# krullgit/3D-Object-Detection-for-autonomous-navigation

Measured on AMD Instinct MI355X. Metric: frames/sec (whole node) + p50 per-frame ms, 16k-pt pillars, higher is better.
Workload: dtype f32 (GEMMs on the 16-bit matrix pipe as split operands -- two float16 pieces per value, 3 products, fp32 accumulate: fp32-equivalent results, measured 1.5e-6 max from the fp32 oracle at this shape)

## Files before the change

3d-object-detection-for-autonomous-navigation_amd/csrc/backbone.hip:

```cpp
#include <stdio.h>
#include <stdlib.h>
#include <string.h>

#include "pp_common.h"

typedef float f32x16 __attribute__((ext_vector_type(16)));
typedef _Float16 f16x8 __attribute__((ext_vector_type(8)));
#define PC_MFMA(A, B, C) __builtin_amdgcn_mfma_f32_32x32x16_f16(A, B, C, 0, 0, 0)
#define PC_PRODUCTS(ACC, XH, XM, YH, YM) \
    ACC = PC_MFMA(XM, YH, ACC); ACC = PC_MFMA(XH, YM, ACC); ACC = PC_MFMA(XH, YH, ACC);
typedef unsigned u32x4 __attribute__((ext_vector_type(4)));

__device__ __forceinline__ float4 buf_load16(__amdgpu_buffer_rsrc_t r, unsigned voff, unsigned soff) {
    const u32x4 v = __builtin_amdgcn_raw_buffer_load_b128(r, voff, soff, 0);
    return make_float4(__uint_as_float(v.x), __uint_as_float(v.y), __uint_as_float(v.z), __uint_as_float(v.w));
}
__device__ __forceinline__ void buf_store16(float4 v, __amdgpu_buffer_rsrc_t r, unsigned voff, unsigned soff) {
    const u32x4 u = {__float_as_uint(v.x), __float_as_uint(v.y), __float_as_uint(v.z), __float_as_uint(v.w)};
    __builtin_amdgcn_raw_buffer_store_b128(u, r, voff, soff, 0);
}
__device__ __forceinline__ __amdgpu_buffer_rsrc_t make_rsrc(const void* base) {
    return __builtin_amdgcn_make_buffer_rsrc(const_cast<void*>(base), 0, 0x7ffffffe, 0x00020000);
}

// ... 464 lines not shown
                const int row = ((it0 + u) * 64 + lane) / ROW4;
                v[u] = *reinterpret_cast<const float4*>(so + row * OSTR + c4 * 4);
                op[u] = s_opix[wave * 32 + row];
            }
#pragma unroll
            for (int u = 0; u < 4; ++u) {
                const int row = ((it0 + u) * 64 + lane) / ROW4;
                if (p0 + wave * 32 + row < a.M)
                    *reinterpret_cast<float4*>(dst + (size_t)(op[u] + delta) * a.ld_out) = v[u];
            }
        }
    }
    if (a.head_mode != 0) {
        f32x16 hacc;
#pragma unroll
        for (int r = 0; r < 16; ++r) hacc[r] = 0.f;
        const float* hA = so + r32 * OSTR + h * (NT / 2);
        const float* hB = a.head_wt + (size_t)r32 * NT + h * (NT / 2);
#pragma unroll
        for (int q = 0; q < NT / 8; ++q) {
            const float4 av = *reinterpret_cast<const float4*>(hA + q * 4);
            const float4 bw = *reinterpret_cast<const float4*>(hB + q * 4);
            hacc = __builtin_amdgcn_mfma_f32_32x32x2f32(av.x, bw.x, hacc, 0, 0, 0);
            hacc = __builtin_amdgcn_mfma_f32_32x32x2f32(av.y, bw.y, hacc, 0, 0, 0);
            hacc = __builtin_amdgcn_mfma_f32_32x32x2f32(av.z, bw.z, hacc, 0, 0, 0);
            hacc = __builtin_amdgcn_mfma_f32_32x32x2f32(av.w, bw.w, hacc, 0, 0, 0);
        }
        const float hb = (a.head_mode == 1) ? a.head_bias[r32] : 0.f;
#pragma unroll
        for (int r = 0; r < 16; ++r) {
            const int prow = wave * 32 + (r & 3) + 8 * (r >> 2) + 4 * h;
            if (p0 + prow < a.M) {
                float* hp = a.head + (size_t)(s_opix[prow] + delta) * PP_HEAD_COLS + r32;
                float v = hacc[r] + hb;
                if (a.head_mode == 2) v += *hp;
                *hp = v;
            }
        }
    }
}


__device__ __forceinline__ float dpp_quad(float v, const int ctrl_xor1) {
    const int x = __float_as_int(v);
    return __int_as_float(ctrl_xor1 ? __builtin_amdgcn_mov_dpp(x, 0xB1, 0xf, 0xf, true)
                                    : __builtin_amdgcn_mov_dpp(x, 0x4E, 0xf, 0xf, true));
}
#define QUAD_XCH(A, B, BIT, XOR1)                          \
    {                                                      \
        const float t_ = (BIT) ? (A) : (B);                \
        const float u_ = dpp_quad(t_, XOR1);               \
        (A) = (BIT) ? u_ : (A);                            \
        (B) = (BIT) ? (B) : u_;                            \
    }
__device__ __forceinline__ void quad_transpose4(float& r0, float& r1, float& r2, float& r3, int lane) {
    const bool b0 = lane & 1, b1 = lane & 2;
    QUAD_XCH(r0, r1, b0, 1)
    QUAD_XCH(r2, r3, b0, 1)
    QUAD_XCH(r0, r2, b1, 0)
    QUAD_XCH(r1, r3, b1, 0)
}

typedef float f32x2_t __attribute__((ext_vector_type(2)));
typedef _Float16 f16x2_t __attribute__((ext_vector_type(2)));
__device__ __forceinline__ void split_f16x2(const float (&v)[8], f16x8& hi, f16x8& mid) {
#pragma unroll
    for (int j = 0; j < 8; j += 2) {
        const f32x2_t x = {v[j], v[j + 1]};
        const f16x2_t h = __builtin_convertvector(x, f16x2_t);
        const f32x2_t r1 = {v[j] - (float)h.x, v[j + 1] - (float)h.y};
        const f16x2_t m = __builtin_convertvector(r1, f16x2_t);
        hi[j] = h.x; hi[j + 1] = h.y;
        mid[j] = m.x; mid[j + 1] = m.y;
    }
}

__device__ __forceinline__ void fast_divmod(int n, int d, float inv_d, int& q, int& r) {
    q = (int)((float)n * inv_d);
    r = n - q * d;
    if (r < 0) { --q; r += d; }
    if (r >= d) { ++q; r -= d; }
}

template <int NT, int S, int WPS, int PREC, int OCC = 0, int TR = 0>
__global__ __launch_bounds__(256, WPS) void k_sep_u(GemmArgs a, int ntiles) {
    static_assert(TR == 0 || (PREC == 1 && OCC == 0), "training forward: split-precision, dense input");
    constexpr bool PW = TR == 2;
    constexpr int NTAP = (TR == 1) ? 11 : 9;
    constexpr int KCH = 16, LSTR = KCH + 4, G = 4;
    constexpr int WW = S + 3;
    constexpr int NLD = PW ? 2 : 3 * WW;
    constexpr int SAW = 32 * LSTR;
    constexpr int SB = (PREC == 0) ? NT * LSTR : PP_NPIECE * NT * 8;
    constexpr int NB4 = (PREC == 0) ? (NT * G + 255) / 256 : (NT * 2 * PP_NPIECE + 255) / 256;
    constexpr int NTILES = NT / 32;
    constexpr int KQ = KCH / 8;
    __shared__ __attribute__((aligned(16))) float smem[8 * SAW + 2 * SB + (PW ? 0 : NTAP * 256) + (TR ? 8 * NT : 0)];
    const int tid = threadIdx.x, lane = tid & 63, wave = tid >> 6;
    float* const sAw = smem + wave * 2 * SAW;
    float* const sB = smem + 8 * SAW;
    float* const sDW = smem + 8 * SAW + 2 * SB;
    [[maybe_unused]] float* const sST = smem + 8 * SAW + 2 * SB + (PW ? 0 : NTAP * 256);

    const int xcd = blockIdx.x & 7, gl = blockIdx.x >> 3, GL = gridDim.x >> 3;
    const int nt_ = ntiles - a.tile_lo;
    const int tbase = a.tile_lo + (int)(((long long)xcd * nt_) >> 3), tend = a.tile_lo + (int)(((long long)(xcd + 1) * nt_) >> 3);
    const int first = tbase + gl;
    const int n0 = blockIdx.y * NT;
    if (first >= tend) {
        if (TR && a.tr_stat != nullptr && tid < 2 * NT)
            a.tr_stat[((size_t)blockIdx.x * 2 + tid / NT) * a.n_total + n0 + tid % NT] = 0.f;
        if (TR && a.tr_stat != nullptr && tid == 0 && blockIdx.y == 0) a.tr_stat[(size_t)gridDim.x * 2 * a.n_total + blockIdx.x] = 0.f;
        return;
    }
    const int ntl = (tend - first + GL - 1) / GL;
    const int cin = a.cin;
    const int nchunks = cin / KCH;
    const int total = ntl * nchunks;

    const int c4 = lane & 3, q = lane >> 2;
    const __amdgpu_buffer_rsrc_t rs_in = make_rsrc(reinterpret_cast<const char*>(a.in) - (PW ? 0 : PP_ZPAD_FLOATS * 4));
    const __amdgpu_buffer_rsrc_t rs_wt = make_rsrc(PREC == 0 ? (const void*)a.wt : (const void*)a.wt16);
    const int hw = a.px_h * a.px_w;
    const float inv_hw = 1.0f / (float)hw, inv_w = 1.0f / (float)a.px_w;
    const int rs4 = a.in_w * cin * 4, cin4 = cin * 4;
    unsigned aoff[NLD];
    [[maybe_unused]] unsigned doff = 0x80000000u;
    [[maybe_unused]] const __amdgpu_buffer_rsrc_t rs_d = make_rsrc(TR ? (const void*)a.tr_D : (const void*)a.in);
    [[maybe_unused]] const bool d_out = TR && a.tr_D != nullptr && blockIdx.y == 0;
    [[maybe_unused]] const bool tr_act = TR && a.tr_coef != nullptr;
#define U_TILE_OFFSETS(TILE)                                                                             \
    {                                                                                                    \
        const int pix0_ = (TILE) * 128 + wave * 32 + 2 * q;                                              \
        const bool pvalid_ = pix0_ < a.M;                                                                \
        if (TR) doff = pvalid_ ? (unsigned)pix0_ * (unsigned)cin4 + (unsigned)(c4 * 16) : 0x80000000u;   \
        const int pc_ = pvalid_ ? pix0_ : 0;                                                             \
        if (PW) {    \
            aoff[0] = pvalid_ ? (unsigned)pc_ * (unsigned)cin4 + (unsigned)(c4 * 16) : 0x80000000u;      \
            aoff[NLD - 1] = pvalid_ ? aoff[0] + (unsigned)cin4 : 0x80000000u;                            \
        } else {                                                                                         \
        int b_, rem_, y_, x0_;                                                                           \
        fast_divmod(pc_, hw, inv_hw, b_, rem_);         \
        fast_divmod(rem_, a.px_w, inv_w, y_, x0_);                                                       \
        const int yi_ = y_ * S - 1, xi_ = x0_ * S - 1;                                                   \
        const unsigned cbase_ =                                                                          \
            (unsigned)(((b_ * a.in_h + y_ * S) * a.in_w + x0_ * S) * cin) * 4u + PP_ZPAD_FLOATS * 4u;    \
                        \
        bool rowok_[3], colok_[WW];                                                                      \
        unsigned rowoff_[3], coloff_[WW];                                                                \
        _Pragma("unroll") for (int dy_ = 0; dy_ < 3; ++dy_) {                                            \
            rowok_[dy_] = pvalid_ & ((unsigned)(yi_ + dy_) < (unsigned)a.in_h);                          \
            rowoff_[dy_] = cbase_ + (unsigned)((dy_ - 1) * rs4);                                         \
        }                                                                                                \
        _Pragma("unroll") for (int dx_ = 0; dx_ < WW; ++dx_) {                                           \
            colok_[dx_] = (unsigned)(xi_ + dx_) < (unsigned)a.in_w;                                      \
            coloff_[dx_] = (unsigned)((dx_ - 1) * cin4);                                                 \
        }                                                                                                \
                                                                       \
        unsigned wbits_[3] = {0u, 0u, 0u};                                                               \
        const bool bits_ = OCC && a.occbits != nullptr;                                     \
        if (bits_) {                                                                                     \
            const unsigned long long* ob_ = a.occbits + (size_t)b_ * a.in_h * a.occ_w64;                 \
            const int pos0_ = xi_ + 1, wi_ = pos0_ >> 6, sh_ = pos0_ & 63;                               \
            _Pragma("unroll") for (int dy_ = 0; dy_ < 3; ++dy_) {                                        \
                const int yy_ = min(max(yi_ + dy_, 0), a.in_h - 1);     \
                const unsigned long long* r_ = ob_ + (size_t)yy_ * a.occ_w64 + wi_;                      \
                const unsigned long long lo_ = r_[0], hi_ = r_[1];                                       \
                wbits_[dy_] = (unsigned)((lo_ >> sh_) | ((hi_ << 1) << (63 - sh_)));                     \
            }                                                                                            \
        }                                                                                                \
        _Pragma("unroll") for (int e = 0; e < NLD; ++e) {                                                \
            const int dy_ = e / WW, dx_ = e % WW;                                                        \
            bool ok_ = rowok_[dy_] & colok_[dx_];                                                        \
            if (OCC) {                                                                                   \
                if (bits_) {                                                                             \
                    ok_ = ok_ & (((wbits_[dy_] >> dx_) & 1u) != 0u);                                     \
                } else {                                                                                 \
                    bool occ_ = false;                                                                   \
                    const int cidx_ = ok_ ? (yi_ + dy_) * a.in_w + xi_ + dx_ : 0;                        \
                    for (int z_ = 0; z_ < a.occ_nz; ++z_)                                                \
                        occ_ = occ_ | (a.occ[(size_t)(b_ * a.occ_nz + z_) * (a.in_h * a.in_w) + cidx_] >= 0); \
                    ok_ = ok_ & occ_;                                                                    \
                }                                                                                        \
            }                                                                                            \
            aoff[e] = (ok_ ? rowoff_[dy_] + coloff_[dx_] : 0u) + (unsigned)(c4 * 16);                    \
        }                                                                                                \
        }                                                                                                \
    }
    constexpr int NBI = (PREC == 0) ? NT * G : NT * 2 * PP_NPIECE;
    unsigned boff[NB4];
    int bdst[NB4];
#pragma unroll
    for (int r = 0; r < NB4; ++r) {
        const int e_ = (tid + 256 * r) % NBI;
        if (PREC == 0) {
            boff[r] = (unsigned)(((n0 + e_ / G) * cin + (e_ % G) * 4) * 4);
            bdst[r] = (e_ / G) * LSTR + (e_ % G) * 4;
        } else {
            const int piece = e_ / (NT * 2), rem = e_ % (NT * 2), row = rem >> 1, half = rem & 1;
            boff[r] = (unsigned)(((piece * a.n_total + n0 + row) * 16 + half * 8) * 2);
            bdst[r] = piece * (NT * 8) + row * 8 + ((half ^ ((row >> 3) & 1)) * 4);
        }
    }
    const unsigned bstep = (PREC == 0) ? (unsigned)(KCH * 4) : (unsigned)(PP_NPIECE * a.n_total * 32);
    float4 rin[NLD];
    float4 rb0, rb1, rb2;
    rb0 = rb1 = rb2 = make_float4(0.f, 0.f, 0.f, 0.f);
    static_assert(NB4 <= 3, "weight prefetch registers");
#define U_LOAD_ACT(KCIDX, RIN)                                                                           \
    {                                                                                                    \
        const unsigned so_ = (unsigned)(KCIDX) * (KCH * 4);                                              \
        _Pragma("unroll") for (int e = 0; e < NLD; ++e) RIN[e] = buf_load16(rs_in, aoff[e], so_);        \
    }
#define U_LOAD_WT(KCIDX)                                                                                 \
    {                                                                                                    \
        const unsigned sb_ = (unsigned)(KCIDX) * bstep;                                                  \
        if (NBI % 256 == 0 || NB4 > 1 || tid < NBI) rb0 = buf_load16(rs_wt, boff[0], sb_);               \
        if (NB4 > 1 && (NBI >= 512 || tid + 256 < NBI)) rb1 = buf_load16(rs_wt, boff[NB4 > 1 ? 1 : 0], sb_);  \
        if (NB4 > 2 && (NBI >= 768 || tid + 512 < NBI)) rb2 = buf_load16(rs_wt, boff[NB4 > 2 ? 2 : 0], sb_);  \
    }
#define U_LOAD_CHUNK(KCIDX) { U_LOAD_ACT(KCIDX, rin) U_LOAD_WT(KCIDX) }
    int ld_tile = first, ld_kc = 0;
    int st_kc = 0;
    int mm_tile = first, mm_kc = 0;
    [[maybe_unused]] float st_n = 0.f;
    U_TILE_OFFSETS(ld_tile)
    U_LOAD_CHUNK(0)
    ld_kc = 1;
    {
        const int ngrp = cin / 4;
        if (!PW) for (int e = tid; e < 9 * ngrp; e += 256) {
            const int t = e / ngrp, g4 = e - t * ngrp;
            reinterpret_cast<float4*>(sDW)[g4 * NTAP + t] = reinterpret_cast<const float4*>(a.dw)[e];
        }
        if (TR) for (int e = tid; e < 8 * NT; e += 256) sST[e] = 0.f;
        if (tr_act) {
            for (int g4 = tid; g4 < ngrp; g4 += 256) {
                const float4 q0 = a.tr_coef[4 * g4], q1 = a.tr_coef[4 * g4 + 1], q2 = a.tr_coef[4 * g4 + 2], q3 = a.tr_coef[4 * g4 + 3];
                reinterpret_cast<float4*>(sDW)[g4 * NTAP + 9] = make_float4(q0.x, q1.x, q2.x, q3.x);
                reinterpret_cast<float4*>(sDW)[g4 * NTAP + 10] = make_float4(q0.y, q1.y, q2.y, q3.y);
            }
        }
    }

    f32x16 acc[NTILES];
#pragma unroll
    for (int n = 0; n < NTILES; ++n)
#pragma unroll
        for (int r = 0; r < 16; ++r) acc[n][r] = 0.f;
    const int h = lane >> 5, r32 = lane & 31;
    float bias_r[NTILES];
#pragma unroll
    for (int n = 0; n < NTILES; ++n) bias_r[n] = (TR && a.bias == nullptr) ? 0.f : a.bias[n0 + n * 32 + r32];
    __syncthreads();

#define U_MFMA(I)                                                                                        \
    if (PREC == 1) {                                                                                     \
        const float* cA = cA0 + ((I) & 1) * SAW;                                                         \
        const float* cB = cB0 + ((I) & 1) * SB;                                                          \
        const float4 a0 = *reinterpret_cast<const float4*>(cA), a1 = *reinterpret_cast<const float4*>(cA + 4);  \
        const float av[8] = {a0.x, a0.y, a0.z, a0.w, a1.x, a1.y, a1.z, a1.w};                            \
        f16x8 ah, am;                                                                                    \
        split_f16x2(av, ah, am);                                                                         \
        _Pragma("unroll") for (int n = 0; n < NTILES; ++n) {                                             \
            const f16x8 bh = *reinterpret_cast<const f16x8*>(cB + n * 32 * 8);                           \
            const f16x8 bm = *reinterpret_cast<const f16x8*>(cB + NT * 8 + n * 32 * 8);                  \
            PC_PRODUCTS(acc[n], ah, am, bh, bm)                                                          \
        }                                                                                                \
    }                                                                                                    \
    if (PREC == 0) {                                                                                     \
        const float* cA = sAw + ((I) & 1) * SAW + r32 * LSTR + h * (KCH / 2);                            \
        const float* cB = sB + ((I) & 1) * SB + r32 * LSTR + h * (KCH / 2);                              \
        float4 a4[KQ];                                                                                   \
        _Pragma("unroll") for (int qq = 0; qq < KQ; ++qq) a4[qq] = *reinterpret_cast<const float4*>(cA + qq * 4);  \
        _Pragma("unroll") for (int n = 0; n < NTILES; ++n) {                                             \
            float4 b4[KQ];                                                                               \
            _Pragma("unroll") for (int qq = 0; qq < KQ; ++qq) b4[qq] = *reinterpret_cast<const float4*>(cB + n * 32 * LSTR + qq * 4);  \
            _Pragma("unroll") for (int qq = 0; qq < KQ; ++qq) {                                          \
                acc[n] = __builtin_amdgcn_mfma_f32_32x32x2f32(a4[qq].x, b4[qq].x, acc[n], 0, 0, 0);      \
                acc[n] = __builtin_amdgcn_mfma_f32_32x32x2f32(a4[qq].y, b4[qq].y, acc[n], 0, 0, 0);      \
                acc[n] = __builtin_amdgcn_mfma_f32_32x32x2f32(a4[qq].z, b4[qq].z, acc[n], 0, 0, 0);      \
                acc[n] = __builtin_amdgcn_mfma_f32_32x32x2f32(a4[qq].w, b4[qq].w, acc[n], 0, 0, 0);      \
            }                                                                                            \
        }                                                                                                \
    }
#define U_STAGE2(P, RIN)                                                                                 \
    {                                                                                                    \
        constexpr int buf = (P) & 1;    \
        float4 o0 = make_float4(0.f, 0.f, 0.f, 0.f), o1 = o0;                                            \
        if (tr_act) {    \
            const float4 sc_ = *reinterpret_cast<const float4*>(twp + 36), sh_ = *reinterpret_cast<const float4*>(twp + 40);  \
            _Pragma("unroll") for (int e = 0; e < NLD; ++e) {                                            \
                RIN[e].x = fmaxf(fmaf(RIN[e].x, sc_.x, sh_.x), 0.f); RIN[e].y = fmaxf(fmaf(RIN[e].y, sc_.y, sh_.y), 0.f);  \
                RIN[e].z = fmaxf(fmaf(RIN[e].z, sc_.z, sh_.z), 0.f); RIN[e].w = fmaxf(fmaf(RIN[e].w, sc_.w, sh_.w), 0.f);  \
            }                                                                                            \
        }                                                                                                \
        if (PW) { o0 = RIN[0]; o1 = RIN[NLD - 1]; }                                                      \
        if (!PW) {                                                                                       \
            const float* tw = twp;                                                                       \
            _Pragma("unroll") for (int dy = 0; dy < 3; ++dy)                                             \
                _Pragma("unroll") for (int dx = 0; dx < 3; ++dx) {                                       \
                    const float4 w4 = *reinterpret_cast<const float4*>(tw + (dy * 3 + dx) * 4);          \
                    const float4 v0 = RIN[PW ? 0 : dy * WW + dx], v1 = RIN[PW ? 0 : dy * WW + S + dx];   \
                    o0.x = fmaf(v0.x, w4.x, o0.x); o0.y = fmaf(v0.y, w4.y, o0.y);                        \
                    o0.z = fmaf(v0.z, w4.z, o0.z); o0.w = fmaf(v0.w, w4.w, o0.w);                        \
                    o1.x = fmaf(v1.x, w4.x, o1.x); o1.y = fmaf(v1.y, w4.y, o1.y);                        \
                    o1.z = fmaf(v1.z, w4.z, o1.z); o1.w = fmaf(v1.w, w4.w, o1.w);                        \
                }                                                                                        \
        }                                                                                                \
        float* dA = sAw + buf * SAW + (2 * q) * LSTR + c4 * 4;                                           \
        *reinterpret_cast<float4*>(dA) = o0;                                                             \
        *reinterpret_cast<float4*>(dA + LSTR) = o1;                                                      \
        if (d_out) {        \
                                                                               \
            const unsigned dv_ = doff + (unsigned)st_kc * (KCH * 4);                                     \
            buf_store16(o0, rs_d, dv_, 0u);                                                              \
            buf_store16(o1, rs_d, dv_ + (unsigned)cin4, 0u);                                             \
        }                                                                                                \
        if (NBI % 256 == 0 || NB4 > 1 || tid < NBI) *reinterpret_cast<float4*>(sB + buf * SB + bdst[0]) = rb0;  \
        if (NB4 > 1 && (NBI >= 512 || tid + 256 < NBI)) *reinterpret_cast<float4*>(sB + buf * SB + bdst[NB4 > 1 ? 1 : 0]) = rb1;  \
        if (NB4 > 2 && (NBI >= 768 || tid + 512 < NBI)) *reinterpret_cast<float4*>(sB + buf * SB + bdst[NB4 > 2 ? 2 : 0]) = rb2;  \
        twp += 4 * (4 * NTAP);                                                                           \
        if (++st_kc == nchunks) { st_kc = 0; twp = sDW + c4 * (4 * NTAP); }                              \
    }
#define U_STAGE(P) U_STAGE2(P, rin)
#define U_ISSUE()                                                                                        \
    {                                                                                                    \
        if (ld_kc == 0) U_TILE_OFFSETS(ld_tile)                                                          \
        U_LOAD_CHUNK(ld_kc)                                                                              \
        if (++ld_kc == nchunks) { ld_kc = 0; ld_tile += GL; }                                            \
    }
#define U_ACT(X) (TR ? (X) : relu_keep_nan(X))
#define U_EPILOGUE()                                                                                     \
    {                                                                                                    \
        const int pw = mm_tile * 128 + wave * 32;                                                        \
        [[maybe_unused]] const int nw = min(max(a.M - pw, 0), 32);    \
        if (TR && nw > 0) {      \
            _Pragma("unroll") for (int n = 0; n < NTILES; ++n) {                                         \
                float s1 = 0.f;                                                                          \
                _Pragma("unroll") for (int r = 0; r < 16; ++r) s1 += acc[n][r];                          \
                s1 += __shfl_xor(s1, 32);                                                                \
                const float mean_ = s1 / (float)nw;                                                      \
                float q = 0.f;                                                                           \
                _Pragma("unroll") for (int r = 0; r < 16; ++r) {                                         \
                    const float dz = acc[n][r] - mean_;                                                  \
                    if (pw + (r & 3) + 8 * (r >> 2) + 4 * h < a.M) q = fmaf(dz, dz, q);                  \
                }                                                                                        \
                q += __shfl_xor(q, 32);                                                                  \
                if (h == 0) {    \
                    float n_ = st_n, s_ = sST[(wave * 2 + 0) * NT + n * 32 + r32], m_ = sST[(wave * 2 + 1) * NT + n * 32 + r32];  \
                    bn_chan_merge(n_, s_, m_, (float)nw, s1, q);                                         \
                    sST[(wave * 2 + 0) * NT + n * 32 + r32] = s_;                                        \
                    sST[(wave * 2 + 1) * NT + n * 32 + r32] = m_;                                        \
                }                                                                                        \
            }                                                                                            \
            st_n += (float)nw;                                                                           \
        }                                                                                                \
        if (pw < a.M) {                                                                                  \
            const int qi = lane & 3, qj = r32 >> 2;                                                      \
            float* dst = a.out + (size_t)(pw + 4 * h + qi) * a.ld_out + a.co_off + n0 + qj * 4;          \
            const bool full = pw + 32 <= a.M;              \
            const int ldo = a.ld_out;                                                                    \
            if (full) {                                                                                  \
                _Pragma("unroll") for (int n = 0; n < NTILES; ++n) {                                     \
                    const float bvn = bias_r[n];                                                         \
                    _Pragma("unroll") for (int g = 0; g < 4; ++g) {                                      \
                        float x0 = U_ACT(acc[n][4 * g + 0] + bvn), x1 = U_ACT(acc[n][4 * g + 1] + bvn);          \
                        float x2 = U_ACT(acc[n][4 * g + 2] + bvn), x3 = U_ACT(acc[n][4 * g + 3] + bvn);          \
                        quad_transpose4(x0, x1, x2, x3, lane);                                           \
                        *reinterpret_cast<float4*>(dst + (8 * g) * ldo + n * 32) = make_float4(x0, x1, x2, x3);  \
                    }                                                                                    \
                }                                                                                        \
            } else {                                                                                     \
                _Pragma("unroll") for (int n = 0; n < NTILES; ++n) {                                     \
                    const float bvn = bias_r[n];                                                         \
                    _Pragma("unroll") for (int g = 0; g < 4; ++g) {                                      \
                        float x0 = U_ACT(acc[n][4 * g + 0] + bvn), x1 = U_ACT(acc[n][4 * g + 1] + bvn);          \
                        float x2 = U_ACT(acc[n][4 * g + 2] + bvn), x3 = U_ACT(acc[n][4 * g + 3] + bvn);          \
                        quad_transpose4(x0, x1, x2, x3, lane);                                           \
                        if (pw + 8 * g + 4 * h + qi < a.M)                                               \
                            *reinterpret_cast<float4*>(dst + (8 * g) * ldo + n * 32) = make_float4(x0, x1, x2, x3);  \
                    }                                                                                    \
                }                                                                                        \
            }                                                                                            \
        }                                                                                                \
        _Pragma("unroll") for (int n = 0; n < NTILES; ++n)                                               \
            _Pragma("unroll") for (int r = 0; r < 16; ++r) acc[n][r] = 0.f;                              \
        mm_kc = 0;                                                                                       \
        mm_tile += GL;                                                                                   \
    }

    const float* twp = sDW + c4 * (4 * NTAP);
    const float* const cA0 = sAw + r32 * LSTR + h * (KCH / 2);
    const float* const cB0 = sB + r32 * 8 + ((h ^ ((r32 >> 3) & 1)) * 4);
    U_STAGE(0)
    U_ISSUE()
    __syncthreads();
    int i = 0;
    for (; i + 3 < total; i += 2) {
        U_MFMA(0)
        U_STAGE(1)
        U_ISSUE()
        if (++mm_kc == nchunks) U_EPILOGUE()
        __syncthreads();
        U_MFMA(1)
        U_STAGE(0)
        U_ISSUE()
        if (++mm_kc == nchunks) U_EPILOGUE()
        __syncthreads();
    }
    U_MFMA(0)
    U_STAGE(1)
    if (++mm_kc == nchunks) U_EPILOGUE()
    __syncthreads();
    U_MFMA(1)
    ++mm_kc;
    U_EPILOGUE()
    if (TR && a.tr_stat != nullptr) {
        __syncthreads();
        const float* red = sST;
        float wn[4] = {0.f, 0.f, 0.f, 0.f};
        for (int t = first; t < tend; t += GL)
#pragma unroll
            for (int w = 0; w < 4; ++w) wn[w] += (float)min(max(a.M - (t * 128 + w * 32), 0), 32);
        if (tid < NT) {
            float n_ = 0.f, s_ = 0.f, m_ = 0.f;
#pragma unroll
            for (int w = 0; w < 4; ++w) bn_chan_merge(n_, s_, m_, wn[w], red[(w * 2) * NT + tid], red[(w * 2 + 1) * NT + tid]);
            a.tr_stat[((size_t)blockIdx.x * 2 + 0) * a.n_total + n0 + tid] = s_;
            a.tr_stat[((size_t)blockIdx.x * 2 + 1) * a.n_total + n0 + tid] = m_;
        }
        if (tid == 0 && blockIdx.y == 0) a.tr_stat[(size_t)gridDim.x * 2 * a.n_total + blockIdx.x] = ((wn[0] + wn[1]) + wn[2]) + wn[3];
    }
#undef U_MFMA
#undef U_STAGE
#undef U_ISSUE
#undef U_EPILOGUE
#undef U_ACT
#undef U_LOAD_CHUNK
#undef U_TILE_OFFSETS
}

constexpr int SEP128_WPB = 2, SEP64_WPB = 3;
constexpr int sep_u_wpc(int nt, int s, bool prec) {
    return s == 1 ? (prec ? (nt == 128 ? SEP128_WPB : (nt == 64 ? SEP64_WPB : 3)) : (nt == 128 ? 3 : 4))
                  : (prec ? (nt == 128 ? 2 : 3) : (nt == 128 ? 2 : (nt == 64 ? 3 : 4)));
}

template <int NT, int S>
static void launch_u(const GemmArgs& a, int n_total, bool prec, bool occ, hipStream_t s) {
    constexpr int WPS = sep_u_wpc(NT, S, false), WPB = sep_u_wpc(NT, S, true);
    const int ntiles = (a.M + 127) / 128;
    const int ny = n_total / NT;
    int slots = (g_num_cus * (prec ? WPB : WPS)) / ny;
    const int mine = ntiles - a.tile_lo;
    int gx = mine < slots ? mine : slots;
    gx = (gx + 7) & ~7;
    dim3 grid((unsigned)gx, ny);
    if (occ)
        PP_LAUNCH("k_sep_u", (k_sep_u<NT, S, WPB, 1, 1>), grid, dim3(256), 0, s, a, ntiles);
    else if (prec)
        PP_LAUNCH("k_sep_u", (k_sep_u<NT, S, WPB, 1>), grid, dim3(256), 0, s, a, ntiles);
    else
        PP_LAUNCH("k_sep_u", (k_sep_u<NT, S, WPS, 0>), grid, dim3(256), 0, s, a, ntiles);
}

int launch_sep_train(const SepTrainArgs& t, hipStream_t s) {
    const long long M = (long long)t.batch * t.out_h * t.out_w;
    const long long in_bytes = (long long)t.batch * t.in_h * t.in_w * t.cin * 4;
    if (t.cin % KC != 0 || t.cout % 32 != 0 || (t.stride != 1 && t.stride != 2) || t.out_w % 2 != 0 || M >= (1 << 24) ||
        in_bytes >= (1ll << 31) - 4096 || M * t.cin * 4 >= (1ll << 31) - 4096 || t.cin > 256)
        return 0;
    GemmArgs a;
    memset(&a, 0, sizeof(a));
    a.in = t.in; a.dw = t.dw; a.wt16 = t.wt16; a.n_total = t.cout; a.out = t.Z;
    a.M = (int)M; a.in_h = t.in_h; a.in_w = t.in_w; a.cin = t.cin; a.px_h = t.out_h; a.px_w = t.out_w;
    a.stride = t.stride; a.ld_out = t.cout; a.co_off = 0; a.cout = t.cout;
    a.tr_coef = t.coef; a.tr_D = t.D; a.tr_stat = t.stat;
    const int ntiles = (a.M + 127) / 128;
    const int nt = (t.cout % 128 == 0) ? 128 : (t.cout % 64 == 0 ? 64 : 32);
    const int ny = t.cout / nt;
    const int wpb = (nt == 128) ? 2 : 3;
    int slots = (g_num_cus * wpb) / ny;
    int gx = ntiles < slots ? ntiles : slots;
    gx = (gx + 7) & ~7;
    const dim3 grid((unsigned)gx, ny);
    const char* tg = t.tag ? t.tag : "k_sep_u_tr";
    if (t.stride == 1) {
        if (nt == 128) PP_LAUNCH(tg, (k_sep_u<128, 1, 2, 1, 0, 1>), grid, dim3(256), 0, s, a, ntiles);
        else if (nt == 64) PP_LAUNCH(tg, (k_sep_u<64, 1, 3, 1, 0, 1>), grid, dim3(256), 0, s, a, ntiles);
        else PP_LAUNCH(tg, (k_sep_u<32, 1, 3, 1, 0, 1>), grid, dim3(256), 0, s, a, ntiles);
    } else {
        if (nt == 128) PP_LAUNCH(tg, (k_sep_u<128, 2, 2, 1, 0, 1>), grid, dim3(256), 0, s, a, ntiles);
        else if (nt == 64) PP_LAUNCH(tg, (k_sep_u<64, 2, 3, 1, 0, 1>), grid, dim3(256), 0, s, a, ntiles);
        else PP_LAUNCH(tg, (k_sep_u<32, 2, 3, 1, 0, 1>), grid, dim3(256), 0, s, a, ntiles);
    }
    return gx;
}

int launch_rows_train(const RowsTrainArgs& t, hipStream_t s) {
    const long long M = t.rows;
    if (t.K % KC != 0 || t.N % 32 != 0 || M % 2 != 0 || M >= (1 << 24) || M * t.K * 4 >= (1ll << 31) - 4096 || t.ld_out % 4 != 0)
        return 0;
    GemmArgs a;
    memset(&a, 0, sizeof(a));
    a.in = t.in; a.wt16 = t.wt16; a.n_total = t.N; a.out = t.out; a.bias = t.bias;
    a.M = (int)M; a.in_h = 1; a.in_w = (int)M; a.cin = t.K; a.px_h = 1; a.px_w = (int)M;
    a.stride = 1; a.ld_out = t.ld_out; a.co_off = 0; a.cout = t.N;
    a.tr_stat = t.stat;
    const int ntiles = (a.M + 127) / 128;
    const int nt = (t.N % 128 == 0) ? 128 : (t.N % 64 == 0 ? 64 : 32);
    const int ny = t.N / nt;
    const int wpb = 3;
    int slots = (g_num_cus * wpb) / ny;
    if (slots < 8) slots = 8;
    int gx = ntiles < slots ? ntiles : slots;
    gx = (gx + 7) & ~7;
    const dim3 grid((unsigned)gx, ny);
    const char* tg = t.tag ? t.tag : "k_sep_u_tr";
    if (nt == 128) PP_LAUNCH(tg, (k_sep_u<128, 1, 3, 1, 0, 2>), grid, dim3(256), 0, s, a, ntiles);
    else if (nt == 64) PP_LAUNCH(tg, (k_sep_u<64, 1, 3, 1, 0, 2>), grid, dim3(256), 0, s, a, ntiles);
    else PP_LAUNCH(tg, (k_sep_u<32, 1, 3, 1, 0, 2>), grid, dim3(256), 0, s, a, ntiles);
    return gx;
}

template <int CO>
__global__ __launch_bounds__(512, 1) void k_sep_p(GemmArgs a, int ntiles) {
    constexpr int KCH = 16, LSTR = KCH + 4, WW = 4, NLD = 12;
    constexpr int SAW = 32 * LSTR;
    constexpr int SB1 = PP_NPIECE * CO * 8;
    constexpr int NTILES = CO / 64;
    constexpr int NB4 = (2 * CO * 2 * PP_NPIECE) / 512;
    __shared__ __attribute__((aligned(16))) float smem[16 * SAW + 4 * SB1 + 9 * 256];
    const int tid = threadIdx.x, lane = tid & 63, wave = tid >> 6;
    const int pg = wave & 3, grp = wave >> 2;
    float* const sA = smem;
    float* const sB = smem + 16 * SAW;
    float* const sDW = smem + 16 * SAW + 4 * SB1;

    const int xcd = blockIdx.x & 7, gl = blockIdx.x >> 3, GL = gridDim.x >> 3;
    const int tbase = (int)(((long long)xcd * ntiles) >> 3), tend = (int)(((long long)(xcd + 1) * ntiles) >> 3);
    const int first = tbase + gl;
    if (first >= tend) return;
    const int ntl = (tend - first + GL - 1) / GL;
    const int cin = a.cin;
    const int npos = cin / (2 * KCH);
    const int total = ntl * npos;

    const int c4 = lane & 3, q = lane >> 2;
    const __amdgpu_buffer_rsrc_t rs_in = make_rsrc(reinterpret_cast<const char*>(a.in) - PP_ZPAD_FLOATS * 4);
    const __amdgpu_buffer_rsrc_t rs_wt = make_rsrc((const void*)a.wt16);
    const int hw = a.px_h * a.px_w;
    const float inv_hw = 1.0f / (float)hw, inv_w = 1.0f / (float)a.px_w;
    const int rs4 = a.in_w * cin * 4, cin4 = cin * 4;
    unsigned aoff[NLD];
#define P_TILE_OFFSETS(TILE)                                                                             \
    {                                                                                                    \
        const int pix0_ = (TILE) * 128 + pg * 32 + 2 * q;                                                \
        const bool pvalid_ = pix0_ < a.M;                                                                \
        const int pc_ = pvalid_ ? pix0_ : 0;                                                             \
        int b_, rem_, y_, x0_;                                                                           \
        fast_divmod(pc_, hw, inv_hw, b_, rem_);                                                          \
        fast_divmod(rem_, a.px_w, inv_w, y_, x0_);                                                       \
        const unsigned cbase_ = (unsigned)(((b_ * a.in_h + y_) * a.in_w + x0_) * cin) * 4u + PP_ZPAD_FLOATS * 4u; \
        bool rowok_[3], colok_[WW];                                                                      \
        _Pragma("unroll") for (int dy_ = 0; dy_ < 3; ++dy_) rowok_[dy_] = pvalid_ & ((unsigned)(y_ - 1 + dy_) < (unsigned)a.in_h); \
        _Pragma("unroll") for (int dx_ = 0; dx_ < WW; ++dx_) colok_[dx_] = (unsigned)(x0_ - 1 + dx_) < (unsigned)a.in_w; \
        _Pragma("unroll") for (int e = 0; e < NLD; ++e) {                                                \
            const int dy_ = e / WW, dx_ = e % WW;                                                        \
            const bool ok_ = rowok_[dy_] & colok_[dx_];                                                  \
            aoff[e] = (ok_ ? cbase_ + (unsigned)((dy_ - 1) * rs4) + (unsigned)((dx_ - 1) * cin4) : 0u) + (unsigned)(c4 * 16); \
        }                                                                                                \
    }
    unsigned boff[NB4];
    int bdst[NB4];
    const unsigned bstep = (unsigned)(PP_NPIECE * a.n_total * 32);
#pragma unroll
    for (int r = 0; r < NB4; ++r) {
        const int e_ = tid + 512 * r;
        const int cc = e_ / (CO * 2 * PP_NPIECE), e2 = e_ % (CO * 2 * PP_NPIECE);
        const int piece = e2 / (CO * 2), rem = e2 % (CO * 2), row = rem >> 1, half = rem & 1;
        boff[r] = (unsigned)(((piece * a.n_total + row) * 16 + half * 8) * 2) + (unsigned)cc * bstep;
        bdst[r] = cc * SB1 + piece * (CO * 8) + row * 8 + ((half ^ ((row >> 3) & 1)) * 4);
    }
    float4 rin[NLD];
    float4 rb[NB4];
#define P_LOAD(POS)                                                                                      \
    {                                                                                                    \
        const unsigned so_ = (unsigned)(2 * (POS) + grp) * (KCH * 4);                                    \
        _Pragma("unroll") for (int e = 0; e < NLD; ++e) rin[e] = buf_load16(rs_in, aoff[e], so_);        \
        const unsigned sb_ = (unsigned)(2 * (POS)) * bstep;                                              \
        _Pragma("unroll") for (int r = 0; r < NB4; ++r) rb[r] = buf_load16(rs_wt, boff[r], sb_);         \
    }
    int ld_tile = first, ld_pos = 0;
    int st_pos = 0;
    int mm_tile = first, mm_pos = 0;
    P_TILE_OFFSETS(ld_tile)
    P_LOAD(0)
    ld_pos = 1;
    {
        const int ngrp = cin / 4;
        for (int e = tid; e < 9 * ngrp; e += 512) {
            const int t = e / ngrp, g4 = e - t * ngrp;
            reinterpret_cast<float4*>(sDW)[g4 * 9 + t] = reinterpret_cast<const float4*>(a.dw)[e];
        }
    }
    f32x16 acc[NTILES];
#pragma unroll
    for (int n = 0; n < NTILES; ++n)
#pragma unroll
        for (int r = 0; r < 16; ++r) acc[n][r] = 0.f;
    const int h = lane >> 5, r32 = lane & 31;
    const int n0 = grp * (CO / 2);
    float bias_r[NTILES];
#pragma unroll
    for (int n = 0; n < NTILES; ++n) bias_r[n] = a.bias[n0 + n * 32 + r32];
    __syncthreads();

    const float* const cA0 = sA + pg * (4 * SAW) + r32 * LSTR + h * (KCH / 2);
    const float* const cB0 = sB + (n0 + r32) * 8 + ((h ^ ((r32 >> 3) & 1)) * 4);
#define P_MFMA(I)                                                                                        \
    {                                                                                                    \
        _Pragma("unroll") for (int c = 0; c < 2; ++c) {                                                  \
            const float* cA = cA0 + (c * 2 + ((I) & 1)) * SAW;                                           \
            const float* cB = cB0 + (((I) & 1) * 2 + c) * SB1;                                           \
            const float4 a0 = *reinterpret_cast<const float4*>(cA), a1 = *reinterpret_cast<const float4*>(cA + 4);  \
            const float av[8] = {a0.x, a0.y, a0.z, a0.w, a1.x, a1.y, a1.z, a1.w};                        \
            f16x8 ah, am;                                                                                \
            split_f16x2(av, ah, am);                                                                     \
            _Pragma("unroll") for (int n = 0; n < NTILES; ++n) {                                         \
                const f16x8 bh = *reinterpret_cast<const f16x8*>(cB + n * 32 * 8);                       \
                const f16x8 bm = *reinterpret_cast<const f16x8*>(cB + CO * 8 + n * 32 * 8);             \
                PC_PRODUCTS(acc[n], ah, am, bh, bm)                                                      \
            }                                                                                            \
        }                                                                                                \
    }
#define P_STAGE(P)                                                                                       \
    {                                                                                                    \
        constexpr int buf = (P) & 1;                                                                     \
        const float* tw = sDW + ((2 * st_pos + grp) * 4 + c4) * 36;                                      \
        float4 o0 = make_float4(0.f, 0.f, 0.f, 0.f), o1 = o0;                                            \
        _Pragma("unroll") for (int dy = 0; dy < 3; ++dy)                                                 \
            _Pragma("unroll") for (int dx = 0; dx < 3; ++dx) {                                           \
                const float4 w4 = *reinterpret_cast<const float4*>(tw + (dy * 3 + dx) * 4);              \
                const float4 v0 = rin[dy * WW + dx], v1 = rin[dy * WW + 1 + dx];                         \
                o0.x = fmaf(v0.x, w4.x, o0.x); o0.y = fmaf(v0.y, w4.y, o0.y);                            \
                o0.z = fmaf(v0.z, w4.z, o0.z); o0.w = fmaf(v0.w, w4.w, o0.w);                            \
                o1.x = fmaf(v1.x, w4.x, o1.x); o1.y = fmaf(v1.y, w4.y, o1.y);                            \
                o1.z = fmaf(v1.z, w4.z, o1.z); o1.w = fmaf(v1.w, w4.w, o1.w);                            \
            }                                                                                            \
        float* dA = sA + pg * (4 * SAW) + (grp * 2 + buf) * SAW + (2 * q) * LSTR + c4 * 4;               \
        *reinterpret_cast<float4*>(dA) = o0;                                                             \
        *reinterpret_cast<float4*>(dA + LSTR) = o1;                                                      \
        _Pragma("unroll") for (int r = 0; r < NB4; ++r)                                                  \
            *reinterpret_cast<float4*>(sB + buf * (2 * SB1) + bdst[r]) = rb[r];                          \
        if (++st_pos == npos) st_pos = 0;                                                                \
    }
#define P_ISSUE()                                                                                        \
    {                                                                                                    \
        if (ld_pos == 0) P_TILE_OFFSETS(ld_tile)                                                         \
        P_LOAD(ld_pos)                                                                                   \
        if (++ld_pos == npos) { ld_pos = 0; ld_tile += GL; }                                             \
    }
#define P_EPILOGUE()                                                                                     \
    {                                                                                                    \
        const int pw = mm_tile * 128 + pg * 32;                                                          \
        if (pw < a.M) {                                                                                  \
            const int qi = lane & 3, qj = r32 >> 2;                                                      \
            float* dst = a.out + (size_t)(pw + 4 * h + qi) * a.ld_out + a.co_off + n0 + qj * 4;          \
            const int ldo = a.ld_out;                                                                    \
            _Pragma("unroll") for (int n = 0; n < NTILES; ++n) {                                         \
                const float bvn = bias_r[n];                                                             \
                _Pragma("unroll") for (int g = 0; g < 4; ++g) {                                          \
                    float x0 = relu_keep_nan(acc[n][4 * g + 0] + bvn), x1 = relu_keep_nan(acc[n][4 * g + 1] + bvn);  \
                    float x2 = relu_keep_nan(acc[n][4 * g + 2] + bvn), x3 = relu_keep_nan(acc[n][4 * g + 3] + bvn);  \
                    quad_transpose4(x0, x1, x2, x3, lane);                                               \
                    if (pw + 8 * g + 4 * h + qi < a.M)                                                   \
                        *reinterpret_cast<float4*>(dst + (8 * g) * ldo + n * 32) = make_float4(x0, x1, x2, x3);  \
                }                                                                                        \
            }                                                                                            \
        }                                                                                                \
        _Pragma("unroll") for (int n = 0; n < NTILES; ++n)                                               \
            _Pragma("unroll") for (int r = 0; r < 16; ++r) acc[n][r] = 0.f;                              \
        mm_pos = 0;                                                                                      \
        mm_tile += GL;                                                                                   \
    }
    P_STAGE(0)
    P_ISSUE()
    __syncthreads();
    int i = 0;
    for (; i + 3 < total; i += 2) {
        P_MFMA(0)
        P_STAGE(1)
        P_ISSUE()
        if (++mm_pos == npos) P_EPILOGUE()
        __syncthreads();
        P_MFMA(1)
        P_STAGE(0)
        P_ISSUE()
        if (++mm_pos == npos) P_EPILOGUE()
        __syncthreads();
    }
    P_MFMA(0)
    P_STAGE(1)
    if (++mm_pos == npos) P_EPILOGUE()
    __syncthreads();
    P_MFMA(1)
    ++mm_pos;
    P_EPILOGUE()
#undef P_MFMA
#undef P_STAGE
#undef P_ISSUE
#undef P_EPILOGUE
#undef P_LOAD
#undef P_TILE_OFFSETS
}

static void launch_p(const GemmArgs& a, hipStream_t s) {
    const int ntiles = (a.M + 127) / 128;
    int gx = ntiles < g_num_cus ? ntiles : g_num_cus;
    gx = (gx + 7) & ~7;
    PP_LAUNCH("k_sep_p", k_sep_p<256>, dim3((unsigned)gx), dim3(512), 0, s, a, ntiles);
}

static bool sep_p_runs(const void* wt16, int stride, int cin, int cout, int n_total, long long M, const int* occ) {
    return wt16 != nullptr && split_precision() && stride == 1 && occ == nullptr && cout == 256 &&
           n_total == 256 && cin % 64 == 0 && cin <= 256 && M < (1 << 24);
}

template <int NT, int S, int NW = 4>
__global__ __launch_bounds__(NW * 64, NW == 4 ? 2 : 1) void k_sep_k4(GemmArgs a) {
    constexpr int KCH = 16, LSTR = KCH + 4;
    constexpr int WW = S + 3, NLD = 3 * WW;
    constexpr int SAW = 32 * LSTR;
    constexpr int SB = PP_NPIECE * NT * 8;
    constexpr int NTILES = NT / 32;
    constexpr int NBL = NT * 2 * PP_NPIECE / 64;
    constexpr int WV = 2 * SAW + 2 * SB;
    static_assert(NW * NTILES * 16 * 64 <= NW * WV, "reduction scratch overlays the staging tiles");
    __shared__ __attribute__((aligned(16))) float smem[NW * WV + 9 * 256];
    const int tid = threadIdx.x, lane = tid & 63, wave = tid >> 6;
    float* const sAw = smem + wave * WV;
    float* const sBw = sAw + 2 * SAW;
    float* const sDW = smem + NW * WV;
    const int n0 = blockIdx.y * NT;
    const int cin = a.cin;
    const int niter = cin / (KCH * NW);

    const int c4 = lane & 3, q = lane >> 2;
    const __amdgpu_buffer_rsrc_t rs_in = make_rsrc(reinterpret_cast<const char*>(a.in) - PP_ZPAD_FLOATS * 4);
    const __amdgpu_buffer_rsrc_t rs_wt = make_rsrc((const void*)a.wt16);
    unsigned aoff[NLD];
    {
        const int hw = a.px_h * a.px_w;
        const int pix0 = blockIdx.x * 32 + 2 * q;
        const bool pvalid = pix0 < a.M;
        const int pc = pvalid ? pix0 : 0;
        const int b = pc / hw, rem = pc - b * hw;
        const int y = rem / a.px_w, x0 = rem - y * a.px_w;
        const int yi = y * S - 1, xi = x0 * S - 1;
        const int rs4 = a.in_w * cin * 4, cin4 = cin * 4;
        const unsigned cbase = (unsigned)(((b * a.in_h + y * S) * a.in_w + x0 * S) * cin) * 4u + PP_ZPAD_FLOATS * 4u;
#pragma unroll
        for (int e = 0; e < NLD; ++e) {
            const int dy = e / WW, dx = e % WW;
            bool ok = pvalid & ((unsigned)(yi + dy) < (unsigned)a.in_h) & ((unsigned)(xi + dx) < (unsigned)a.in_w);
            if (a.occ != nullptr) {
                bool occ = false;
                const int cidx = ok ? (yi + dy) * a.in_w + xi + dx : 0;
                for (int z = 0; z < a.occ_nz; ++z)
                    occ = occ | (a.occ[(size_t)(b * a.occ_nz + z) * (a.in_h * a.in_w) + cidx] >= 0);
                ok = ok & occ;
            }
            aoff[e] = (ok ? cbase + (unsigned)((dy - 1) * rs4 + (dx - 1) * cin4) : 0u) + (unsigned)(c4 * 16);
        }
    }
    unsigned boff[NBL];
    int bdst[NBL];
#pragma unroll
    for (int r = 0; r < NBL; ++r) {
        const int e = lane + 64 * r;
        const int piece = e / (NT * 2), rem = e % (NT * 2), row = rem >> 1, half = rem & 1;
        boff[r] = (unsigned)(((piece * a.n_total + n0 + row) * 16 + half * 8) * 2);
        bdst[r] = piece * (NT * 8) + row * 8 + ((half ^ ((row >> 3) & 1)) * 4);
    }
    const unsigned bstep = (unsigned)(PP_NPIECE * a.n_total * 32);
    float4 rin[NLD];
    float4 rb[NBL];
#define K4_LOAD(KC)                                                                                      \
    {                                                                                                    \
        const unsigned so_ = (unsigned)(KC) * (KCH * 4), sb_ = (unsigned)(KC) * bstep;                   \
        _Pragma("unroll") for (int e = 0; e < NLD; ++e) rin[e] = buf_load16(rs_in, aoff[e], so_);        \
        _Pragma("unroll") for (int r = 0; r < NBL; ++r) rb[r] = buf_load16(rs_wt, boff[r], sb_);         \
    }
#define K4_STAGE(KC, BUF)                                                                                \
    {                                                                                                    \
        const float* tw = sDW + ((KC) * 4 + c4) * 36;                                                    \
        float4 o0 = make_float4(0.f, 0.f, 0.f, 0.f), o1 = o0;                                            \
        _Pragma("unroll") for (int dy = 0; dy < 3; ++dy)                                                 \
            _Pragma("unroll") for (int dx = 0; dx < 3; ++dx) {                                           \
                const float4 w4 = *reinterpret_cast<const float4*>(tw + (dy * 3 + dx) * 4);              \
                const float4 v0 = rin[dy * WW + dx], v1 = rin[dy * WW + S + dx];                         \
                o0.x = fmaf(v0.x, w4.x, o0.x); o0.y = fmaf(v0.y, w4.y, o0.y);                            \
                o0.z = fmaf(v0.z, w4.z, o0.z); o0.w = fmaf(v0.w, w4.w, o0.w);                            \
                o1.x = fmaf(v1.x, w4.x, o1.x); o1.y = fmaf(v1.y, w4.y, o1.y);                            \
// ... 1016 lines not shown
```

Before: 92280.

## Share depthwise 3x3 window columns across lanes via DPP row shifts

For stride-1 dense inference depthwise convolution, each lane now loads only its two own columns plus one halo column (only edge lanes of each 4-lane group actually load), and gets neighbouring columns from adjacent lanes through DPP row_shr/row_shl by 4. Per-lane global loads drop from 12 to 9 slots with fewer active, which cuts memory traffic and VGPR pressure in the staging path. This depends on pixel rows being 8-aligned and on the lane-to-pixel mapping matching the DPP shift pattern. The new path is enabled only when the shape checks pass, and a wrong lane mapping would give incorrect halo values.

```diff
diff --git a/3d-object-detection-for-autonomous-navigation_amd/csrc/backbone.hip b/3d-object-detection-for-autonomous-navigation_amd/csrc/backbone.hip
--- a/3d-object-detection-for-autonomous-navigation_amd/csrc/backbone.hip
+++ b/3d-object-detection-for-autonomous-navigation_amd/csrc/backbone.hip
@@ -570,14 +570,41 @@
     if (r >= d) { ++q; r -= d; }
 }
 
-template <int NT, int S, int WPS, int PREC, int OCC = 0, int TR = 0>
+__device__ __forceinline__ float dpp_row_shr4(float old, float src) {
+    return __int_as_float(__builtin_amdgcn_update_dpp(__float_as_int(old), __float_as_int(src), 0x114, 0xf, 0xf, false));
+}
+__device__ __forceinline__ float dpp_row_shl4(float old, float src) {
+    return __int_as_float(__builtin_amdgcn_update_dpp(__float_as_int(old), __float_as_int(src), 0x104, 0xf, 0xf, false));
+}
+#define SEP_SHARED_WINDOW(WIN, C0, C1, H)                                                                \
+    {                                                                                                    \
+        WIN[0] = make_float4(dpp_row_shr4(H.x, C1.x), dpp_row_shr4(H.y, C1.y), dpp_row_shr4(H.z, C1.z), dpp_row_shr4(H.w, C1.w)); \
+        WIN[1] = C0;                                                                                     \
+        WIN[2] = C1;                                                                                     \
+        WIN[3] = make_float4(dpp_row_shl4(H.x, C0.x), dpp_row_shl4(H.y, C0.y), dpp_row_shl4(H.z, C0.z), dpp_row_shl4(H.w, C0.w)); \
+    }
+#define SEP_SHARED_OFFSETS(AOFF, Q, ROWOK, COLOK, ROWOFF, CIN4, C4)                                      \
+    {                                                                                                    \
+        const int qm_ = (Q) & 3;                                                                         \
+        const bool hcol_ = qm_ == 0 ? COLOK[0] : COLOK[3];                                               \
+        const bool hload_ = (qm_ == 0) | (qm_ == 3);                                                     \
+        const unsigned hoff_ = qm_ == 0 ? 0u - (unsigned)(CIN4) : 2u * (unsigned)(CIN4);                 \
+        _Pragma("unroll") for (int dy_ = 0; dy_ < 3; ++dy_) {                                            \
+            AOFF[dy_ * 3 + 0] = ((ROWOK[dy_] & COLOK[1]) ? ROWOFF[dy_] : 0u) + (unsigned)((C4) * 16);    \
+            AOFF[dy_ * 3 + 1] = ((ROWOK[dy_] & COLOK[2]) ? ROWOFF[dy_] + (unsigned)(CIN4) : 0u) + (unsigned)((C4) * 16); \
+            AOFF[dy_ * 3 + 2] = hload_ ? ((ROWOK[dy_] & hcol_) ? ROWOFF[dy_] + hoff_ : 0u) + (unsigned)((C4) * 16) : 0x80000000u; \
+        }                                                                                                \
+    }
+
+template <int NT, int S, int WPS, int PREC, int OCC = 0, int TR = 0, int SH = 0>
 __global__ __launch_bounds__(256, WPS) void k_sep_u(GemmArgs a, int ntiles) {
     static_assert(TR == 0 || (PREC == 1 && OCC == 0), "training forward: split-precision, dense input");
+    static_assert(SH == 0 || (S == 1 && PREC == 1 && OCC == 0 && TR == 0), "shared window: stride 1, dense input, inference");
     constexpr bool PW = TR == 2;
     constexpr int NTAP = (TR == 1) ? 11 : 9;
     constexpr int KCH = 16, LSTR = KCH + 4, G = 4;
     constexpr int WW = S + 3;
-    constexpr int NLD = PW ? 2 : 3 * WW;
+    constexpr int NLD = PW ? 2 : (SH ? 9 : 3 * WW);
     constexpr int SAW = 32 * LSTR;
     constexpr int SB = (PREC == 0) ? NT * LSTR : PP_NPIECE * NT * 8;
     constexpr int NB4 = (PREC == 0) ? (NT * G + 255) / 256 : (NT * 2 * PP_NPIECE + 255) / 256;
@@ -657,6 +684,9 @@
                 wbits_[dy_] = (unsigned)((lo_ >> sh_) | ((hi_ << 1) << (63 - sh_)));                     \
             }                                                                                            \
         }                                                                                                \
+        if constexpr (SH != 0) {                                                                         \
+            SEP_SHARED_OFFSETS(aoff, q, rowok_, colok_, rowoff_, cin4, c4)                               \
+        } else {                                                                                         \
         _Pragma("unroll") for (int e = 0; e < NLD; ++e) {                                                \
             const int dy_ = e / WW, dx_ = e % WW;                                                        \
             bool ok_ = rowok_[dy_] & colok_[dx_];                                                        \
@@ -672,6 +702,7 @@
                 }                                                                                        \
             }                                                                                            \
             aoff[e] = (ok_ ? rowoff_[dy_] + coloff_[dx_] : 0u) + (unsigned)(c4 * 16);                    \
+        }                                                                                                \
         }                                                                                                \
         }                                                                                                \
     }
@@ -786,15 +817,19 @@
         if (PW) { o0 = RIN[0]; o1 = RIN[NLD - 1]; }                                                      \
         if (!PW) {                                                                                       \
             const float* tw = twp;                                                                       \
-            _Pragma("unroll") for (int dy = 0; dy < 3; ++dy)                                             \
+            _Pragma("unroll") for (int dy = 0; dy < 3; ++dy) {                                           \
+                [[maybe_unused]] float4 win_[4];                                                         \
+                if constexpr (SH != 0) SEP_SHARED_WINDOW(win_, RIN[dy * 3], RIN[dy * 3 + 1], RIN[dy * 3 + 2]) \
                 _Pragma("unroll") for (int dx = 0; dx < 3; ++dx) {                                       \
                     const float4 w4 = *reinterpret_cast<const float4*>(tw + (dy * 3 + dx) * 4);          \
-                    const float4 v0 = RIN[PW ? 0 : dy * WW + dx], v1 = RIN[PW ? 0 : dy * WW + S + dx];   \
+                    const float4 v0 = SH ? win_[dx] : RIN[(PW || SH) ? 0 : dy * WW + dx];                \
+                    const float4 v1 = SH ? win_[dx + 1] : RIN[(PW || SH) ? 0 : dy * WW + S + dx];        \
                     o0.x = fmaf(v0.x, w4.x, o0.x); o0.y = fmaf(v0.y, w4.y, o0.y);                        \
                     o0.z = fmaf(v0.z, w4.z, o0.z); o0.w = fmaf(v0.w, w4.w, o0.w);                        \
                     o1.x = fmaf(v1.x, w4.x, o1.x); o1.y = fmaf(v1.y, w4.y, o1.y);                        \
                     o1.z = fmaf(v1.z, w4.z, o1.z); o1.w = fmaf(v1.w, w4.w, o1.w);                        \
                 }                                                                                        \
+            }                                                                                            \
         }                                                                                                \
         float* dA = sAw + buf * SAW + (2 * q) * LSTR + c4 * 4;                                           \
         *reinterpret_cast<float4*>(dA) = o0;                                                             \
@@ -935,6 +970,10 @@
                   : (prec ? (nt == 128 ? 2 : 3) : (nt == 128 ? 2 : (nt == 64 ? 3 : 4)));
 }
 
+static bool sep_shared_window(const GemmArgs& a) {
+    return a.stride == 1 && a.px_w % 8 == 0 && a.in_w == a.px_w && a.in_h == a.px_h;
+}
+
 template <int NT, int S>
 static void launch_u(const GemmArgs& a, int n_total, bool prec, bool occ, hipStream_t s) {
     constexpr int WPS = sep_u_wpc(NT, S, false), WPB = sep_u_wpc(NT, S, true);
@@ -945,12 +984,19 @@
     int gx = mine < slots ? mine : slots;
     gx = (gx + 7) & ~7;
     dim3 grid((unsigned)gx, ny);
-    if (occ)
+    if (occ) {
         PP_LAUNCH("k_sep_u", (k_sep_u<NT, S, WPB, 1, 1>), grid, dim3(256), 0, s, a, ntiles);
-    else if (prec)
+    } else if (prec) {
+        if constexpr (S == 1 && NT == 64) {
+            if (sep_shared_window(a)) {
+                PP_LAUNCH("k_sep_u", (k_sep_u<NT, S, WPB, 1, 0, 0, 1>), grid, dim3(256), 0, s, a, ntiles);
+                return;
+            }
+        }
         PP_LAUNCH("k_sep_u", (k_sep_u<NT, S, WPB, 1>), grid, dim3(256), 0, s, a, ntiles);
-    else
+    } else {
         PP_LAUNCH("k_sep_u", (k_sep_u<NT, S, WPS, 0>), grid, dim3(256), 0, s, a, ntiles);
+    }
 }
 
 int launch_sep_train(const SepTrainArgs& t, hipStream_t s) {
@@ -1012,9 +1058,9 @@
     return gx;
 }
 
-template <int CO>
+template <int CO, int SH = 0>
 __global__ __launch_bounds__(512, 1) void k_sep_p(GemmArgs a, int ntiles) {
-    constexpr int KCH = 16, LSTR = KCH + 4, WW = 4, NLD = 12;
+    constexpr int KCH = 16, LSTR = KCH + 4, WW = 4, NLD = SH ? 9 : 12;
     constexpr int SAW = 32 * LSTR;
     constexpr int SB1 = PP_NPIECE * CO * 8;
     constexpr int NTILES = CO / 64;
@@ -1054,10 +1100,15 @@
         bool rowok_[3], colok_[WW];                                                                      \
         _Pragma("unroll") for (int dy_ = 0; dy_ < 3; ++dy_) rowok_[dy_] = pvalid_ & ((unsigned)(y_ - 1 + dy_) < (unsigned)a.in_h); \
         _Pragma("unroll") for (int dx_ = 0; dx_ < WW; ++dx_) colok_[dx_] = (unsigned)(x0_ - 1 + dx_) < (unsigned)a.in_w; \
+        if constexpr (SH != 0) {                                                                         \
+            const unsigned rowoff_[3] = {cbase_ - (unsigned)rs4, cbase_, cbase_ + (unsigned)rs4};        \
+            SEP_SHARED_OFFSETS(aoff, q, rowok_, colok_, rowoff_, cin4, c4)                               \
+        } else {                                                                                         \
         _Pragma("unroll") for (int e = 0; e < NLD; ++e) {                                                \
             const int dy_ = e / WW, dx_ = e % WW;                                                        \
             const bool ok_ = rowok_[dy_] & colok_[dx_];                                                  \
             aoff[e] = (ok_ ? cbase_ + (unsigned)((dy_ - 1) * rs4) + (unsigned)((dx_ - 1) * cin4) : 0u) + (unsigned)(c4 * 16); \
+        }                                                                                                \
         }                                                                                                \
     }
     unsigned boff[NB4];
@@ -1128,15 +1179,19 @@
         constexpr int buf = (P) & 1;                                                                     \
         const float* tw = sDW + ((2 * st_pos + grp) * 4 + c4) * 36;                                      \
         float4 o0 = make_float4(0.f, 0.f, 0.f, 0.f), o1 = o0;                                            \
-        _Pragma("unroll") for (int dy = 0; dy < 3; ++dy)                                                 \
+        _Pragma("unroll") for (int dy = 0; dy < 3; ++dy) {                                               \
+            [[maybe_unused]] float4 win_[4];                                                             \
+            if constexpr (SH != 0) SEP_SHARED_WINDOW(win_, rin[dy * 3], rin[dy * 3 + 1], rin[dy * 3 + 2]) \
             _Pragma("unroll") for (int dx = 0; dx < 3; ++dx) {                                           \
                 const float4 w4 = *reinterpret_cast<const float4*>(tw + (dy * 3 + dx) * 4);              \
-                const float4 v0 = rin[dy * WW + dx], v1 = rin[dy * WW + 1 + dx];                         \
+                const float4 v0 = SH ? win_[dx] : rin[SH ? 0 : dy * WW + dx];                            \
+                const float4 v1 = SH ? win_[dx + 1] : rin[SH ? 0 : dy * WW + 1 + dx];                    \
                 o0.x = fmaf(v0.x, w4.x, o0.x); o0.y = fmaf(v0.y, w4.y, o0.y);                            \
                 o0.z = fmaf(v0.z, w4.z, o0.z); o0.w = fmaf(v0.w, w4.w, o0.w);                            \
                 o1.x = fmaf(v1.x, w4.x, o1.x); o1.y = fmaf(v1.y, w4.y, o1.y);                            \
                 o1.z = fmaf(v1.z, w4.z, o1.z); o1.w = fmaf(v1.w, w4.w, o1.w);                            \
             }                                                                                            \
+        }                                                                                                \
         float* dA = sA + pg * (4 * SAW) + (grp * 2 + buf) * SAW + (2 * q) * LSTR + c4 * 4;               \
         *reinterpret_cast<float4*>(dA) = o0;                                                             \
         *reinterpret_cast<float4*>(dA + LSTR) = o1;                                                      \
@@ -1208,7 +1263,8 @@
     const int ntiles = (a.M + 127) / 128;
     int gx = ntiles < g_num_cus ? ntiles : g_num_cus;
     gx = (gx + 7) & ~7;
-    PP_LAUNCH("k_sep_p", k_sep_p<256>, dim3((unsigned)gx), dim3(512), 0, s, a, ntiles);
+    if (sep_shared_window(a)) PP_LAUNCH("k_sep_p", (k_sep_p<256, 1>), dim3((unsigned)gx), dim3(512), 0, s, a, ntiles);
+    else PP_LAUNCH("k_sep_p", k_sep_p<256>, dim3((unsigned)gx), dim3(512), 0, s, a, ntiles);
 }
 
 static bool sep_p_runs(const void* wt16, int stride, int cin, int cout, int n_total, long long M, const int* occ) {
```

Result: faster. 94020 (median of 6 runs) (+1.9%).
